# MathsionYang/Ransac

Measured on NVIDIA B200. Metric: hypothesis x point evaluations/s (useful, whole job); ms per robust fit in config, higher is better.
Workload: dtype f32

## Files before the change

### ransac_b200/csrc/common.cuh

```cuda
#pragma once
#include <cuda_runtime.h>
#include <stdint.h>

#include "../../include/usac_gpu.h"

#define USAC_REC_STRIDE 32
#define USAC_TILE_PAIRS 128
#ifndef USAC_WARP_STAGES
#define USAC_WARP_STAGES 2
#endif
#define USAC_SCORE_THREADS 128
#ifndef USAC_SCORE_MIN_CTAS
#define USAC_SCORE_MIN_CTAS 4
#endif
#ifndef USAC_SCORE_GRID_CTAS
#define USAC_SCORE_GRID_CTAS USAC_SCORE_MIN_CTAS
#endif
#ifndef USAC_SQ_MIN_CTAS
#define USAC_SQ_MIN_CTAS 5
#endif
#ifndef USAC_PPI
#define USAC_PPI 4
#endif

enum { REC_MODEL = 0, REC_HINV = 9, REC_BAND = 18, REC_THR = 22 };

struct ProblemDesc {
    int n;
    int n_pairs;
    long long aos_off;
    long long pair_off;
    float mx1, my1, mx2, my2;
    int neigh_type, knn;
    long long knn_off;
    long long grid_off;
    long long cell_start_off;
    long long growth_off, term_off, pool_off;
    long long cursor_off;
    unsigned long long pn_len;
};

__host__ __device__ __forceinline__ unsigned long long pnapsac_length(const ProblemDesc& pd) {
    return pd.pn_len ? pd.pn_len : 20ull * (unsigned long long)pd.n;
}

struct FitState {
    float best_model[9];
    int best_cnt;
    float best_sum;
    long long best_hyp;
    int best_midx;
    unsigned iters, max_iters, samples_drawn, rounds;
    int done;
    int round_pending;
    unsigned long long evals, useful_evals;
    unsigned prosac_t, prosac_n, prosac_largest, prosac_term_len;
    unsigned prosac_t_next, prosac_n_next, prosac_largest_next;
    double sprt_eps, sprt_delta, sprt_A;
    unsigned sprt_cursor;
    int sprt_last_update, sprt_ntests;
};

#define CUDA_TRY(ctx, expr)                                                                         \
    do {                                                                                            \
        cudaError_t _e = (expr);                                                                    \
        if (_e != cudaSuccess) { (ctx)->set_error(#expr, cudaGetErrorString(_e)); return USAC_ERR_CUDA; } \
    } while (0)

__host__ __device__ __forceinline__ int usac_sample_size(int est) {
    return est == USAC_EST_LINE2D ? 2 : est == USAC_EST_HOMOGRAPHY ? 4 : est == USAC_EST_FUNDAMENTAL ? 7 : 5;
}
__host__ __device__ __forceinline__ int usac_models_per_sample(int est) { return est == USAC_EST_FUNDAMENTAL ? 3 : 1; }
__host__ __device__ __forceinline__ constexpr int usac_point_dim(int est) { return est == USAC_EST_LINE2D ? 2 : 4; }

__host__ __device__ __forceinline__ void philox4x32_10(uint32_t c0, uint32_t c1, uint32_t c2, uint32_t c3, uint32_t k0, uint32_t k1, uint32_t out[4]) {
#pragma unroll
    for (int r = 0; r < 10; r++) {
        const uint64_t p0 = (uint64_t)0xD2511F53u * c0, p1 = (uint64_t)0xCD9E8D57u * c2;
        const uint32_t n0 = (uint32_t)(p1 >> 32) ^ c1 ^ k0, n1 = (uint32_t)p1, n2 = (uint32_t)(p0 >> 32) ^ c3 ^ k1, n3 = (uint32_t)p0;
        c0 = n0; c1 = n1; c2 = n2; c3 = n3;
        k0 += 0x9E3779B9u; k1 += 0xBB67AE85u;
    }
    out[0] = c0; out[1] = c1; out[2] = c2; out[3] = c3;
}

__host__ __device__ __forceinline__ void philox_unique(uint64_t seed, uint64_t hyp, uint32_t stream, int n, int m, int* out) {
    uint32_t w[8];
    for (int blk = 0; blk * 4 < m; blk++)
        philox4x32_10((uint32_t)hyp, (uint32_t)(hyp >> 32), (uint32_t)blk, stream, (uint32_t)seed, (uint32_t)(seed >> 32), w + 4 * blk);
    int sorted[8];
    for (int i = 0; i < m; i++) {
        int j = (int)(((uint64_t)w[i] * (uint64_t)(uint32_t)(n - i)) >> 32);
        int pos = 0;
        while (pos < i && j >= sorted[pos]) { j++; pos++; }
        for (int q = i; q > pos; q--) sorted[q] = sorted[q - 1];
        sorted[pos] = j;
        out[i] = j;
    }
}

__device__ __forceinline__ unsigned long long score_key(int cnt, float sum) {
    const unsigned s = (sum > 0.f) ? __float_as_uint(sum) : 0u;
// ... 3 lines not shown
```

### ransac_b200/csrc/score.cuh

```cuda
#pragma once
#include "strict_math.cuh"

__device__ __forceinline__ float fast_rcp(float x) { float r; asm("rcp.approx.ftz.f32 %0, %1;" : "=f"(r) : "f"(x)); return r; }
__device__ __forceinline__ float fast_sqrt(float x) { float r; asm("sqrt.approx.ftz.f32 %0, %1;" : "=f"(r) : "f"(x)); return r; }
__device__ __forceinline__ float fast_rsqrt(float x) { float r; asm("rsqrt.approx.ftz.f32 %0, %1;" : "=f"(r) : "f"(x)); return r; }
__device__ __forceinline__ float2 dup(float x) { return make_float2(x, x); }
__device__ __forceinline__ float abs_max_nan(float a, float b) { float r; asm("max.NaN.f32 %0, %1, %2;" : "=f"(r) : "f"(fabsf(a)), "f"(fabsf(b))); return r; }

__device__ __forceinline__ uint32_t smem_u32(const void* p) { return (uint32_t)__cvta_generic_to_shared(p); }
__device__ __forceinline__ void mbar_init(uint64_t* bar, uint32_t count) {
    asm volatile("mbarrier.init.shared::cta.b64 [%0], %1;" ::"r"(smem_u32(bar)), "r"(count));
}
__device__ __forceinline__ void mbar_expect_tx(uint64_t* bar, uint32_t bytes) {
    asm volatile("mbarrier.arrive.expect_tx.shared::cta.b64 _, [%0], %1;" ::"r"(smem_u32(bar)), "r"(bytes) : "memory");
}
__device__ __forceinline__ bool mbar_try_wait(uint64_t* bar, uint32_t parity) {
    uint32_t ok;
    asm volatile(
        "{\n\t.reg .pred p;\n\t"
        "mbarrier.try_wait.parity.shared::cta.b64 p, [%1], %2;\n\t"
        "selp.u32 %0, 1, 0, p;\n\t}"
        : "=r"(ok)
        : "r"(smem_u32(bar)), "r"(parity)
        : "memory");
    return ok != 0;
}
__device__ __forceinline__ void mbar_wait(uint64_t* bar, uint32_t parity) {
    while (!mbar_try_wait(bar, parity)) {}
}
__device__ __forceinline__ void bulk_copy_g2s(void* dst_smem, const void* src_gmem, uint32_t bytes, uint64_t* bar) {
    asm volatile("cp.async.bulk.shared::cluster.global.mbarrier::complete_tx::bytes [%0], [%1], %2, [%3];" ::"r"(smem_u32(dst_smem)),
                 "l"(src_gmem), "r"(bytes), "r"(smem_u32(bar))
                 : "memory");
}


template <int EST> struct FastModel;

template <> struct FastModel<USAC_EST_HOMOGRAPHY> {
    static constexpr bool WEIGHTED = false;
    float a11, a12, a13, a21, a22, a23, h31, h32, h33;
    float b11, b12, b13, b21, b22, b23, g31, g32, g33;
    float negT, k1, k2;
    __device__ __forceinline__ void load(const float* r) {
        a11 = -r[0]; a12 = -r[1]; a13 = -r[2]; a21 = -r[3]; a22 = -r[4]; a23 = -r[5]; h31 = r[6]; h32 = r[7]; h33 = r[8];
        b11 = -r[9]; b12 = -r[10]; b13 = -r[11]; b21 = -r[12]; b22 = -r[13]; b23 = -r[14]; g31 = r[15]; g32 = r[16]; g33 = r[17];
        negT = -2.f * r[REC_THR]; k1 = r[REC_BAND]; k2 = r[REC_BAND + 1];
        T2p = 2.f * r[REC_THR] * 1.0000019f;
    }
    static constexpr bool TWO_PHASE = true;
    float T2p;
    struct P1 { float2 sa, nz; };
    __device__ __forceinline__ void phase1(const float4 A, const float4 B, P1& s) const {
        const float2 X1 = make_float2(A.x, A.y), Y1 = make_float2(A.z, A.w), X2 = make_float2(B.x, B.y), Y2 = make_float2(B.z, B.w);
        const float2 nz = __ffma2_rn(dup(h31), X1, __ffma2_rn(dup(h32), Y1, dup(h33)));
        const float2 nx = __ffma2_rn(dup(a11), X1, __ffma2_rn(dup(a12), Y1, dup(a13)));
        const float2 ny = __ffma2_rn(dup(a21), X1, __ffma2_rn(dup(a22), Y1, dup(a23)));
        const float2 ax = __ffma2_rn(X2, nz, nx), ay = __ffma2_rn(Y2, nz, ny);
        s.sa = __ffma2_rn(ay, ay, __fmul2_rn(ax, ax));
        s.nz = nz;
    }
    __device__ __forceinline__ void sure(const P1& s, bool& ox, bool& oy) const {
        const float2 az = make_float2(fabsf(s.nz.x), fabsf(s.nz.y));
        const float2 c = __ffma2_rn(dup(T2p), az, dup(k1));
        const float2 c2 = __fmul2_rn(c, c);
        ox = s.sa.x > c2.x; oy = s.sa.y > c2.y;
    }
    __device__ __forceinline__ void phase2(const float4 A, const float4 B, const P1& s, float2& t, float2& band) const {
        const float2 X1 = make_float2(A.x, A.y), Y1 = make_float2(A.z, A.w), X2 = make_float2(B.x, B.y), Y2 = make_float2(B.z, B.w);
        const float2 r1 = make_float2(fabsf(fast_rcp(s.nz.x)), fabsf(fast_rcp(s.nz.y)));
        const float2 d1 = __fmul2_rn(make_float2(fast_sqrt(s.sa.x), fast_sqrt(s.sa.y)), r1);
        const float2 mz = __ffma2_rn(dup(g31), X2, __ffma2_rn(dup(g32), Y2, dup(g33)));
        const float2 mx = __ffma2_rn(dup(b11), X2, __ffma2_rn(dup(b12), Y2, dup(b13)));
        const float2 my = __ffma2_rn(dup(b21), X2, __ffma2_rn(dup(b22), Y2, dup(b23)));
        const float2 r2 = make_float2(fast_rcp(mz.x), fast_rcp(mz.y));
        const float2 ex = __ffma2_rn(mx, r2, X1), ey = __ffma2_rn(my, r2, Y1);
        const float2 sb = __ffma2_rn(ey, ey, __fmul2_rn(ex, ex));
        const float2 d2 = make_float2(fast_sqrt(sb.x), fast_sqrt(sb.y));
        t = __fadd2_rn(__fadd2_rn(d1, dup(negT)), d2);
        const float2 p2 = __fmul2_rn(dup(k2), r2);
        band = __ffma2_rn(dup(k1), r1, make_float2(fabsf(p2.x), fabsf(p2.y)));
    }
    __device__ __forceinline__ void eval(const float4 A, const float4 B, float2& t, float2& s, float2& w) const {
        P1 st;
        bool ox, oy;
        phase1(A, B, st);
        sure(st, ox, oy);
        phase2(A, B, st, t, s);
        if (ox) { t.x = 1.f; s.x = 0.f; }
        if (oy) { t.y = 1.f; s.y = 0.f; }
        w = t;
    }
    __device__ __forceinline__ float2 reject(const float4 A, const float4 B, float2& bound) const {
        const float2 X1 = make_float2(A.x, A.y), Y1 = make_float2(A.z, A.w), X2 = make_float2(B.x, B.y), Y2 = make_float2(B.z, B.w);
        const float2 nz = __ffma2_rn(dup(h31), X1, __ffma2_rn(dup(h32), Y1, dup(h33)));
        const float2 nx = __ffma2_rn(dup(a11), X1, __ffma2_rn(dup(a12), Y1, dup(a13)));
        const float2 ny = __ffma2_rn(dup(a21), X1, __ffma2_rn(dup(a22), Y1, dup(a23)));
        const float2 ax = __ffma2_rn(X2, nz, nx), ay = __ffma2_rn(Y2, nz, ny);
        bound = __ffma2_rn(dup(T2p), make_float2(fabsf(nz.x), fabsf(nz.y)), dup(k1));
        return make_float2(abs_max_nan(ax.x, ay.x), abs_max_nan(ax.y, ay.y));
    }
    static __device__ __forceinline__ float finish(float sum_em, int cnt, float thr) { return 0.5f * (sum_em + (float)cnt * (2.f * thr)); }
    static __device__ __forceinline__ float strict_to_em(float err, float thr) { return 2.f * err - 2.f * thr; }
};

template <> struct FastModel<USAC_EST_FUNDAMENTAL> {
#ifdef USAC_F_SINGLE_PHASE
    static constexpr bool TWO_PHASE = false;
#else
    static constexpr bool TWO_PHASE = true;
#endif
    static constexpr bool WEIGHTED = true;
    float f11, f12, f13, f21, f22, f23, f31, f32, f33, negthr, b1, b0, negthrP, b0P;
    __device__ __forceinline__ void load(const float* r) {
        f11 = r[0]; f12 = r[1]; f13 = r[2]; f21 = r[3]; f22 = r[4]; f23 = r[5]; f31 = r[6]; f32 = r[7]; f33 = r[8];
        negthr = -r[REC_THR]; b1 = r[REC_BAND]; b0 = r[REC_BAND + 1];
        negthrP = -(r[REC_THR] + b1) * 1.0000039f;
        b0P = b0 * 1.0000039f + 1e-37f;
    }
    struct P1 { float2 n2, den; };
    __device__ __forceinline__ void phase1(const float4 A, const float4 B, P1& s) const {
        const float2 X1 = make_float2(A.x, A.y), Y1 = make_float2(A.z, A.w), X2 = make_float2(B.x, B.y), Y2 = make_float2(B.z, B.w);
        const float2 a = __ffma2_rn(dup(f11), X1, __ffma2_rn(dup(f12), Y1, dup(f13)));
        const float2 b = __ffma2_rn(dup(f21), X1, __ffma2_rn(dup(f22), Y1, dup(f23)));
        const float2 c = __ffma2_rn(dup(f11), X2, __ffma2_rn(dup(f21), Y2, dup(f31)));
        const float2 d = __ffma2_rn(dup(f12), X2, __ffma2_rn(dup(f22), Y2, dup(f32)));
        const float2 n = __ffma2_rn(X2, a, __ffma2_rn(Y2, b, __ffma2_rn(dup(f31), X1, __ffma2_rn(dup(f32), Y1, dup(f33)))));
        s.n2 = __fmul2_rn(n, n);
        s.den = __ffma2_rn(d, d, __ffma2_rn(c, c, __ffma2_rn(b, b, __fmul2_rn(a, a))));
    }
    __device__ __forceinline__ void sure(const P1& s, bool& ox, bool& oy) const {
        const float2 u = __ffma2_rn(dup(negthrP), s.den, s.n2);
        ox = u.x > b0P; oy = u.y > b0P;
    }
    __device__ __forceinline__ void phase2(const float4, const float4, const P1& s, float2& t, float2& band) const {
        t = __ffma2_rn(dup(negthr), s.den, s.n2);
        band = __ffma2_rn(dup(b1), s.den, dup(b0));
    }
    __device__ __forceinline__ float2 weight(const P1& s) const { return make_float2(fast_rcp(s.den.x), fast_rcp(s.den.y)); }
    __device__ __forceinline__ float2 reject(const float4 A, const float4 B, float2& bound) const {
        bound = make_float2(0.f, 0.f);
        const float2 X1 = make_float2(A.x, A.y), Y1 = make_float2(A.z, A.w), X2 = make_float2(B.x, B.y), Y2 = make_float2(B.z, B.w);
        const float2 a = __ffma2_rn(dup(f11), X1, __ffma2_rn(dup(f12), Y1, dup(f13)));
        const float2 b = __ffma2_rn(dup(f21), X1, __ffma2_rn(dup(f22), Y1, dup(f23)));
        const float2 c = __ffma2_rn(dup(f11), X2, __ffma2_rn(dup(f21), Y2, dup(f31)));
        const float2 d = __ffma2_rn(dup(f12), X2, __ffma2_rn(dup(f22), Y2, dup(f32)));
        const float2 cp = __ffma2_rn(dup(f31), X1, __ffma2_rn(dup(f32), Y1, dup(f33)));
        const float2 n = __ffma2_rn(X2, a, __ffma2_rn(Y2, b, cp));
        const float2 den = __ffma2_rn(d, d, __ffma2_rn(c, c, __ffma2_rn(b, b, __fmul2_rn(a, a))));
        return __ffma2_rn(dup(negthrP), den, __ffma2_rn(n, n, dup(-b0P)));
    }
    __device__ __forceinline__ void eval(const float4 A, const float4 B, float2& t, float2& s, float2& w) const {
        P1 st;
        phase1(A, B, st);
        phase2(A, B, st, t, s);
        w = weight(st);
    }
    static __device__ __forceinline__ float finish(float sum_em, int cnt, float thr) { return sum_em + (float)cnt * thr; }
    static __device__ __forceinline__ float strict_to_em(float err, float thr) { return err - thr; }
};

template <> struct FastModel<USAC_EST_ESSENTIAL> {
    static constexpr bool WEIGHTED = false;
    float e11, e12, e13, e21, e22, e23, e31, e32, e33, negT, ka, kb, k0, negka, C2;
    __device__ __forceinline__ void load(const float* r) {
        e11 = r[0]; e12 = r[1]; e13 = r[2]; e21 = r[3]; e22 = r[4]; e23 = r[5]; e31 = r[6]; e32 = r[7]; e33 = r[8];
        negT = -2.f * r[REC_THR]; ka = r[REC_BAND]; kb = r[REC_BAND + 1]; k0 = r[REC_BAND + 2];
        negka = -ka;
        const float c = (2.f * r[REC_THR] + k0) * 1.0000039f;
        C2 = c * c * 1.0000039f;
    }
    __device__ __forceinline__ float2 reject(const float4 A, const float4 B, float2& bound) const {
        bound = make_float2(0.f, 0.f);
        const float2 X1 = make_float2(A.x, A.y), Y1 = make_float2(A.z, A.w), X2 = make_float2(B.x, B.y), Y2 = make_float2(B.z, B.w);
        const float2 l1 = __ffma2_rn(dup(e11), X2, __ffma2_rn(dup(e21), Y2, dup(e31)));
        const float2 l2 = __ffma2_rn(dup(e12), X2, __ffma2_rn(dup(e22), Y2, dup(e32)));
        const float2 l3 = __ffma2_rn(dup(e13), X2, __ffma2_rn(dup(e23), Y2, dup(e33)));
        const float2 a1 = __ffma2_rn(l1, X1, __ffma2_rn(l2, Y1, l3));
        const float2 a2 = __ffma2_rn(l2, l2, __fmul2_rn(l1, l1));
        const float2 v = __fadd2_rn(make_float2(fabsf(a1.x), fabsf(a1.y)), dup(negka));
        const float2 m = __fmul2_rn(dup(C2), a2);
        return __ffma2_rn(v, make_float2(fabsf(v.x), fabsf(v.y)), make_float2(-m.x, -m.y));
    }
// ... 422 lines not shown
```

### ransac_b200/csrc/score_sq.cuh

```cuda
#pragma once
#include "score.cuh"

#ifndef USAC_SQ_TRIPVOTE
#define USAC_SQ_TRIPVOTE 2
#endif
#ifndef USAC_SQ_PREFETCH
#define USAC_SQ_PREFETCH 0
#endif
#define USAC_SQ_LANE_CAP 16
#define USAC_SQ_FIXED_BITS 36
#define USAC_SQ_LO_BITS 22

__device__ __forceinline__ void sq_push(bool pred, uint32_t& qaddr, uint32_t entry) {
    asm volatile(
        "{\n\t.reg .pred p;\n\t"
        "setp.ne.u32 p, %1, 0;\n\t"
        "@p st.shared.u32 [%0], %2;\n\t"
        "@p add.u32 %0, %0, 128;\n\t}"
        : "+r"(qaddr)
        : "r"((uint32_t)pred), "r"(entry));
}

template <int EST>
__device__ __noinline__ void sq_drain(const uint32_t* __restrict__ q, uint32_t cnt, uint32_t* pre, const float* __restrict__ recs_group,
                                      const float* __restrict__ aos, int n, double scale, uint32_t* mcnt, uint32_t* mlo, uint32_t* mhi) {
    const int lane = threadIdx.x & 31;
    uint32_t incl = cnt;
#pragma unroll
    for (int o = 1; o < 32; o <<= 1) { const uint32_t y = __shfl_up_sync(0xffffffffu, incl, o); if (lane >= o) incl += y; }
    const uint32_t total = __shfl_sync(0xffffffffu, incl, 31);
    pre[lane] = incl - cnt;
    __syncwarp();
    for (uint32_t base = 0; base < total; base += 64) {
        int l[2], idx[2];
        bool on[2];
        float4 p[2];
#pragma unroll
        for (int h = 0; h < 2; h++) {
            const uint32_t t = base + 32u * h + lane;
            on[h] = t < total;
            l[h] = 0; idx[h] = 0;
            if (on[h]) {
                int ll = 0;
#pragma unroll
                for (int step = 16; step; step >>= 1) if (pre[ll + step] <= t) ll += step;
                l[h] = ll;
                idx[h] = (int)q[(t - pre[ll]) * 32 + ll];
                on[h] = idx[h] < n;
            }
            p[h] = make_float4(0.f, 0.f, 0.f, 0.f);
            if (on[h]) {
                if (EST == USAC_EST_LINE2D) { const float2 v = reinterpret_cast<const float2*>(aos)[idx[h]]; p[h] = make_float4(v.x, v.y, 0.f, 0.f); }
                else p[h] = reinterpret_cast<const float4*>(aos)[idx[h]];
            }
        }
#pragma unroll
        for (int h = 0; h < 2; h++) {
            if (!on[h]) continue;
            const float* rec = recs_group + (size_t)l[h] * USAC_REC_STRIDE;
            const float err = strict_error<EST>(rec, p[h].x, p[h].y, p[h].z, p[h].w);
            if (err < rec[REC_THR]) {
                const unsigned long long fix = __double2ull_rn((double)err * scale);
                atomicAdd(&mcnt[l[h]], 1u);
                atomicAdd(&mlo[l[h]], (uint32_t)(fix & ((1u << USAC_SQ_LO_BITS) - 1u)));
                atomicAdd(&mhi[l[h]], (uint32_t)(fix >> USAC_SQ_LO_BITS));
            }
        }
    }
}

template <int EST>
__global__ void __launch_bounds__(USAC_SCORE_THREADS, USAC_SQ_MIN_CTAS) score_sq_kernel(const ScoreArgs a) {
    constexpr int PAIR_FLOATS = (EST == USAC_EST_LINE2D) ? 4 : 8;
    constexpr int NWARPS = USAC_SCORE_THREADS / 32;
    static_assert(USAC_SQ_LANE_CAP >= 4 * USAC_PPI, "a lane's queue must hold two trips of pushes");
    __shared__ __align__(128) float tile_all[NWARPS][USAC_WARP_STAGES][USAC_TILE_PAIRS * PAIR_FLOATS];
    __shared__ __align__(8) uint64_t full_all[NWARPS][USAC_WARP_STAGES];
    __shared__ __align__(128) uint32_t queue_all[NWARPS][USAC_SQ_LANE_CAP * 32];
    __shared__ uint32_t macc_all[NWARPS][4][32];

    const int lane = threadIdx.x & 31, warp = threadIdx.x >> 5;
    float (*tile)[USAC_TILE_PAIRS * PAIR_FLOATS] = tile_all[warp];
    uint64_t* full = full_all[warp];
    uint32_t* queue = queue_all[warp];
    uint32_t* mcnt = macc_all[warp][0];
    uint32_t* mlo = macc_all[warp][1];
    uint32_t* mhi = macc_all[warp][2];
    uint32_t* pre = macc_all[warp][3];
    const uint32_t q_first = smem_u32(queue) + 4u * (uint32_t)lane;
    const uint32_t q_limit = q_first + 128u * (USAC_SQ_LANE_CAP - 2 * USAC_PPI);
    if (lane == 0) {
#pragma unroll
        for (int s = 0; s < USAC_WARP_STAGES; s++) mbar_init(&full[s], 1);
        asm volatile("fence.mbarrier_init.release.cluster;" ::: "memory");
        asm volatile("fence.proxy.async.shared::cta;" ::: "memory");
    }
    __syncwarp();

    const int mgroups = a.mblocks * NWARPS;
    const unsigned total = a.items ? *a.item_count : (unsigned)a.slots * (unsigned)a.nchunks * (unsigned)mgroups;
    uint32_t g = 0;

    unsigned pending = 0;
    if (USAC_SQ_PREFETCH && lane == 0) pending = atomicAdd(a.work, 1u) - a.work_base;
    for (;;) {
        if (!USAC_SQ_PREFETCH && lane == 0) pending = atomicAdd(a.work, 1u) - a.work_base;
        const unsigned item = __shfl_sync(0xffffffffu, pending, 0);
        int slot, chunk, mgroup;
        if (!score_item(a, item, total, mgroups, slot, chunk, mgroup)) break;
        if (USAC_SQ_PREFETCH && lane == 0) pending = atomicAdd(a.work, 1u) - a.work_base;
        const int M = a.mvalid ? a.mvalid[slot] : a.M;
        if (mgroup * 32 >= M) continue;
        const ProblemDesc pd = a.prob[a.active ? a.active[slot] : slot];
        const int m = mgroup * 32 + lane;
        const bool live = m < M;
        const float* recs_group = a.recs + ((size_t)slot * a.mstride + (size_t)mgroup * 32) * USAC_REC_STRIDE;
        const float* rec = recs_group + (size_t)(live ? lane : 0) * USAC_REC_STRIDE;
        const size_t out = ((size_t)slot * a.nchunks + chunk) * a.mstride + m;

        const int pair_begin = chunk * a.chunk_pairs;
        const int npairs = min(pair_begin + a.chunk_pairs, pd.n_pairs) - pair_begin;
        if (npairs <= 0) {
            if (live) { a.part_cnt[out] = 0; a.part_sum[out] = 0.f; }
            continue;
        }
        const int ntiles = (npairs + USAC_TILE_PAIRS - 1) / USAC_TILE_PAIRS;
        const float* src = a.pairs + ((size_t)pd.pair_off + pair_begin) * PAIR_FLOATS;

        if (lane == 0) {
            asm volatile("fence.proxy.async.shared::cta;" ::: "memory");
            for (int k = 0; k < USAC_WARP_STAGES && k < ntiles; k++) {
                const int s = (g + k) % USAC_WARP_STAGES;
                const uint32_t bytes = min(USAC_TILE_PAIRS, npairs - k * USAC_TILE_PAIRS) * PAIR_FLOATS * 4;
                mbar_expect_tx(&full[s], bytes);
                bulk_copy_g2s(tile[s], src + (size_t)k * USAC_TILE_PAIRS * PAIR_FLOATS, bytes, &full[s]);
            }
        }
        mcnt[lane] = 0u; mlo[lane] = 0u; mhi[lane] = 0u;
        uint32_t acc_cnt = 0;
        unsigned long long acc_sum = 0;
        __syncwarp();

        FastModel<EST> fm;
        fm.load(rec);
        const float thr = rec[REC_THR];
        const double scale = (double)(1ull << USAC_SQ_FIXED_BITS) / (double)thr;
        const float* aos = a.aos + (size_t)pd.aos_off * (EST == USAC_EST_LINE2D ? 2 : 4);
        uint32_t qaddr = q_first;

        auto drain = [&]() {
            asm volatile("" ::: "memory");
            __syncwarp();
            sq_drain<EST>(queue, (qaddr - q_first) >> 7, pre, recs_group, aos, pd.n, scale, mcnt, mlo, mhi);
            __syncwarp();
            acc_cnt += mcnt[lane];
            acc_sum += ((unsigned long long)mhi[lane] << USAC_SQ_LO_BITS) + mlo[lane];
            mcnt[lane] = 0u; mlo[lane] = 0u; mhi[lane] = 0u;
            qaddr = q_first;
            __syncwarp();
        };

        for (int k = 0; k < ntiles; k++) {
            const int s = (g + k) % USAC_WARP_STAGES;
            mbar_wait(&full[s], ((g + k) / USAC_WARP_STAGES) & 1);
            const int np = min(USAC_TILE_PAIRS, npairs - k * USAC_TILE_PAIRS);
            const float4* tp = reinterpret_cast<const float4*>(tile[s]);
            uint32_t ebase = (uint32_t)(2 * (pair_begin + k * USAC_TILE_PAIRS));
            auto load_pair = [&](int j, float4& A, float4& B) {
                if (EST == USAC_EST_LINE2D) { A = tp[j]; B = A; }
                else { A = tp[2 * j]; B = tp[2 * j + 1]; }
            };
            int j = 0;
#pragma unroll 1
            for (; j + USAC_PPI <= np; j += USAC_PPI) {
                float2 z[USAC_PPI], zb[USAC_PPI];
#pragma unroll
                for (int q = 0; q < USAC_PPI; q++) {
                    float4 A, B;
                    load_pair(j + q, A, B);
                    z[q] = fm.reject(A, B, zb[q]);
                }
                bool lane_any = false;
#pragma unroll
                for (int q = 0; q < USAC_PPI; q++) lane_any = lane_any || !(z[q].x > zb[q].x) || !(z[q].y > zb[q].y);
                if (!USAC_SQ_TRIPVOTE || (EST != USAC_EST_HOMOGRAPHY && USAC_SQ_TRIPVOTE == 2) || __any_sync(0xffffffffu, lane_any && live)) {
#pragma unroll
                    for (int q = 0; q < USAC_PPI; q++) {
                        sq_push(!(z[q].x > zb[q].x) && live, qaddr, ebase + 2 * q);
                        sq_push(!(z[q].y > zb[q].y) && live, qaddr, ebase + 2 * q + 1);
                    }
                    if (__any_sync(0xffffffffu, qaddr > q_limit)) drain();
                }
                ebase += 2 * USAC_PPI;
            }
            if (j < np) {
                const int rest = np - j;
#pragma unroll
                for (int q = 0; q < USAC_PPI; q++) {
                    if (q < rest) {
                        float4 A, B;
                        load_pair(j + q, A, B);
                        float2 zb;
                        const float2 z = fm.reject(A, B, zb);
                        sq_push(!(z.x > zb.x) && live, qaddr, ebase + 2 * q);
                        sq_push(!(z.y > zb.y) && live, qaddr, ebase + 2 * q + 1);
                    }
                }
                if (__any_sync(0xffffffffu, qaddr > q_limit)) drain();
            }
            __syncwarp();
            if (lane == 0 && k + USAC_WARP_STAGES < ntiles) {
                asm volatile("fence.proxy.async.shared::cta;" ::: "memory");
                const int nk = k + USAC_WARP_STAGES;
                const uint32_t bytes = min(USAC_TILE_PAIRS, npairs - nk * USAC_TILE_PAIRS) * PAIR_FLOATS * 4;
                mbar_expect_tx(&full[s], bytes);
                bulk_copy_g2s(tile[s], src + (size_t)nk * USAC_TILE_PAIRS * PAIR_FLOATS, bytes, &full[s]);
            }
        }
        g += (uint32_t)ntiles;
        if (__any_sync(0xffffffffu, qaddr != q_first)) drain();
        if (live) {
            a.part_cnt[out] = (int)acc_cnt;
            a.part_sum[out] = (float)((double)acc_sum / scale);
        }
        __syncwarp();
    }
}
```

### ransac_b200/csrc/usac_gpu.cu

```cuda
#include <dlfcn.h>

#include <cub/device/device_radix_sort.cuh>
#include <cub/device/device_scan.cuh>

#include <algorithm>
#include <chrono>
#include <cmath>
#include <cstdio>
#include <cstdlib>
#include <cstring>
#include <map>
#include <string>
#include <thread>
#include <tuple>
#include <vector>

#include "essential.cuh"
#include "pipeline.cuh"
#include "score.cuh"
#include "score_sq.cuh"
#include "sprt.cuh"
#include "refit.cuh"
#include "lo.cuh"
#include "knn.cuh"
// ... 543 lines not shown
    CUDA_TRY(c, cudaStreamSynchronize(c->stream));
    *k_out = d.knn;
    return USAC_OK;
}

extern "C" int usac_gpu_set_pnapsac_length(usac_gpu_ctx* c, int problem, unsigned long long local_samples) {
    if (!c || problem < 0 || problem >= c->P) return fail(c, USAC_ERR_ARG, "set_pnapsac_length: bad arguments");
    cudaSetDevice(c->device);
    c->h_prob[problem].pn_len = local_samples;
    return push_desc(c);
}

extern "C" int usac_gpu_set_neighbors_grid(usac_gpu_ctx* c, int problem, int cell_size) {
    if (!c || problem < 0 || problem >= c->P || cell_size <= 0) return fail(c, USAC_ERR_ARG, "set_neighbors_grid: bad arguments");
    if (usac_point_dim(c->est) != 4) return fail(c, USAC_ERR_ARG, "set_neighbors_grid: needs correspondences (nearest_neighbors.cpp:172 reads 4 columns)");
    cudaSetDevice(c->device);
    ProblemDesc& d = c->h_prob[problem];
    const int n = d.n;
    SideUsed& u = c->side;
    CUDA_TRY(c, reserve_segment(c->d_cell_of_point, u.grid, (size_t)n, c->stream));
    CUDA_TRY(c, reserve_segment(c->d_members, u.grid, (size_t)n, c->stream));
    CUDA_TRY(c, reserve_segment(c->d_rank, u.grid, (size_t)n, c->stream));
    CUDA_TRY(c, reserve_segment(c->d_cell_start, u.cell_start, (size_t)n + 1, c->stream));
    CUDA_TRY(c, c->d_grid_keys.ensure(2 * (size_t)n));
    CUDA_TRY(c, c->d_grid_ints.ensure(4 * (size_t)n + 1));
    struct { unsigned long long* p; } keys{c->d_grid_keys.p}, skeys{c->d_grid_keys.p + n};
    struct { int* p; } idx{c->d_grid_ints.p}, sidx{c->d_grid_ints.p + n}, flags{c->d_grid_ints.p + 2 * (size_t)n}, cellid1{c->d_grid_ints.p + 3 * (size_t)n},
        ovf{c->d_grid_ints.p + 4 * (size_t)n};
    CUDA_TRY(c, cudaMemsetAsync(ovf.p, 0, sizeof(int), c->stream));
    const int g = (n + 255) / 256;
    grid_keys_kernel<<<g, 256, 0, c->stream>>>(c->d_aos.p + (size_t)d.aos_off * 4, n, (float)cell_size, keys.p, idx.p, ovf.p);
    size_t tb1 = 0, tb2 = 0;
    cub::DeviceRadixSort::SortPairs(nullptr, tb1, keys.p, skeys.p, idx.p, sidx.p, n, 0, 64, c->stream);
    cub::DeviceScan::InclusiveSum(nullptr, tb2, flags.p, cellid1.p, n, c->stream);
    CUDA_TRY(c, c->d_grid_temp.ensure(std::max(tb1, tb2)));
    struct { unsigned char* p; } temp{c->d_grid_temp.p};
    size_t tb = std::max(tb1, tb2);
    CUDA_TRY(c, cub::DeviceRadixSort::SortPairs(temp.p, tb, keys.p, skeys.p, idx.p, sidx.p, n, 0, 64, c->stream));
    grid_flags_kernel<<<g, 256, 0, c->stream>>>(skeys.p, n, flags.p);
    tb = std::max(tb1, tb2);
    CUDA_TRY(c, cub::DeviceScan::InclusiveSum(temp.p, tb, flags.p, cellid1.p, n, c->stream));
    int* cs = c->d_cell_start.p + u.cell_start;
    grid_fill_tail_kernel<<<(n + 1 + 255) / 256, 256, 0, c->stream>>>(cellid1.p, n, cs);
    grid_starts_kernel<<<g, 256, 0, c->stream>>>(flags.p, cellid1.p, n - 0, cs);
    grid_scatter_kernel<<<g, 256, 0, c->stream>>>(sidx.p, cellid1.p, cs, n, c->d_cell_of_point.p + u.grid, c->d_members.p + u.grid, c->d_rank.p + u.grid);
    int h_ovf = 0;
    CUDA_TRY(c, cudaMemcpyAsync(&h_ovf, ovf.p, sizeof(int), cudaMemcpyDeviceToHost, c->stream));
    CUDA_TRY(c, cudaStreamSynchronize(c->stream));
    CUDA_TRY(c, cudaGetLastError());
    if (h_ovf) return fail(c, USAC_ERR_ARG, "set_neighbors_grid: cell coordinates exceed 16 bits (cell_size too small for this coordinate range)");
    d.grid_off = (long long)u.grid;
    d.cell_start_off = (long long)u.cell_start;
    u.grid += (size_t)n;
    u.cell_start += (size_t)n + 1;
    if (d.cursor_off < 0) CUDA_TRY(c, append_segment(c->d_cursors, u.cursors, (const unsigned*)nullptr, 3 * (size_t)n + 1, &d.cursor_off, c->stream));
    d.neigh_type = USAC_NEIGH_GRID;
    return push_desc(c);
}

extern "C" int usac_gpu_set_sprt_pool(usac_gpu_ctx* c, int problem, const int* pool) {
    if (!c || problem < 0 || problem >= c->P || !pool) return fail(c, USAC_ERR_ARG, "set_sprt_pool: bad arguments");
    cudaSetDevice(c->device);
    SideUsed& u = c->side;
    ProblemDesc& d = c->h_prob[problem];
    for (int i = 0; i < d.n; i++) if (pool[i] < 0 || pool[i] >= d.n) return fail(c, USAC_ERR_ARG, "set_sprt_pool: index out of range");
    CUDA_TRY(c, append_segment(c->d_pool, u.pool, pool, (size_t)d.n, &d.pool_off, c->stream));
    const int dim = usac_point_dim(c->est);
    CUDA_TRY(c, c->d_pool_pts.ensure((size_t)c->total_points * dim));
    pool_gather_kernel<<<(d.n + 255) / 256, 256, 0, c->stream>>>(c->d_aos.p + (size_t)d.aos_off * dim, c->d_pool.p + d.pool_off, d.n, dim,
                                                                  c->d_pool_pts.p + (size_t)d.aos_off * dim);
    CUDA_TRY(c, cudaGetLastError());
    c->h_pool_set[problem] = 1;
    return push_desc(c);
}

static void launch_score(usac_gpu_ctx* c, ScoreArgs a, int slots, int mblocks, bool dense_survivors = false) {
    a.mblocks = mblocks; a.slots = slots;
    constexpr int warps_per_cta = USAC_SCORE_THREADS / 32;
    const long long items = (long long)slots * a.nchunks * mblocks * warps_per_cta;
    const unsigned grid = (unsigned)std::min<long long>((items + warps_per_cta - 1) / warps_per_cta,
                                                        (long long)c->prop.multiProcessorCount * USAC_SCORE_GRID_CTAS);
    static const int legacy = [] { const char* e = getenv("USAC_GPU_SCORE_LEGACY"); return e ? atoi(e) : 0; }();
    const bool loop_kernel = legacy == 1 || c->est == USAC_EST_LINE2D || (dense_survivors && legacy != 2);
    unsigned grid_ctas = grid;
    if (a.items) {
        grid_ctas = (unsigned)c->prop.multiProcessorCount * (loop_kernel ? USAC_SCORE_GRID_CTAS : USAC_SQ_MIN_CTAS);
        a.work = c->d_item_count.p + 1; a.work_base = 0;
    } else {
        if (!loop_kernel) grid_ctas = (unsigned)std::min<long long>((items + warps_per_cta - 1) / warps_per_cta, (long long)c->prop.multiProcessorCount * USAC_SQ_MIN_CTAS);
        a.work = c->d_work.p; a.work_base = c->work_next;
        c->work_next += (unsigned)items + grid_ctas * warps_per_cta;
    }
    auto& ev = c->next_score_event();
    cudaEventRecord(ev.first, c->stream);
    if (loop_kernel) {
        switch (c->est) {
            case USAC_EST_LINE2D: score_kernel<USAC_EST_LINE2D><<<grid_ctas, USAC_SCORE_THREADS, 0, c->stream>>>(a); break;
            case USAC_EST_HOMOGRAPHY: score_kernel<USAC_EST_HOMOGRAPHY><<<grid_ctas, USAC_SCORE_THREADS, 0, c->stream>>>(a); break;
            case USAC_EST_FUNDAMENTAL: score_kernel<USAC_EST_FUNDAMENTAL><<<grid_ctas, USAC_SCORE_THREADS, 0, c->stream>>>(a); break;
            default: score_kernel<USAC_EST_ESSENTIAL><<<grid_ctas, USAC_SCORE_THREADS, 0, c->stream>>>(a); break;
        }
    } else {
        switch (c->est) {
            case USAC_EST_HOMOGRAPHY: score_sq_kernel<USAC_EST_HOMOGRAPHY><<<grid_ctas, USAC_SCORE_THREADS, 0, c->stream>>>(a); break;
            case USAC_EST_FUNDAMENTAL: score_sq_kernel<USAC_EST_FUNDAMENTAL><<<grid_ctas, USAC_SCORE_THREADS, 0, c->stream>>>(a); break;
            default: score_sq_kernel<USAC_EST_ESSENTIAL><<<grid_ctas, USAC_SCORE_THREADS, 0, c->stream>>>(a); break;
        }
    }
    if (!a.items && cudaPeekAtLastError() != cudaSuccess) c->work_next = a.work_base;
    cudaEventRecord(ev.second, c->stream);
    c->last_launches++;
    c->last_score_launches++;
}

static void plan_chunks(const usac_gpu_ctx* c, int slots, int mblocks, int max_pairs, int* chunk_pairs, int* nchunks) {
    static const int per_warp = [] { const char* e = getenv("USAC_GPU_ITEMS_PER_WARP"); const int v = e ? atoi(e) : 0; return v > 0 ? v : 16; }();
    const long long warps = (long long)c->prop.multiProcessorCount * std::max(USAC_SCORE_GRID_CTAS, USAC_SQ_MIN_CTAS) * (USAC_SCORE_THREADS / 32);
    const long long base = (long long)slots * mblocks * (USAC_SCORE_THREADS / 32);
    static const int min_tiles_env = [] { const char* e = getenv("USAC_GPU_MIN_TILES"); return e ? atoi(e) : 0; }();
    const int min_tiles = min_tiles_env > 0 ? min_tiles_env : (max_pairs >= 65536 ? 8 : 2);
    const int max_chunks = std::min(65535, std::max(1, max_pairs / (min_tiles * USAC_TILE_PAIRS)));
    int nc = (int)std::min<long long>((per_warp * warps + base - 1) / base, max_chunks);
    nc = std::max(nc, 1);
    int cp = (max_pairs + nc - 1) / nc;
    cp = ((cp + 1) / 2) * 2;
    nc = (max_pairs + cp - 1) / cp;
    *chunk_pairs = cp;
    *nchunks = std::max(nc, 1);
}

static void collect_timing(usac_gpu_ctx* c) {
    float ms = 0;
    cudaEventElapsedTime(&ms, c->ev0, c->ev1);
    c->last_total_ms = ms;
    float s = 0;
    for (size_t i = 0; i < c->score_events_used; i++) {
        float t = 0;
        cudaEventElapsedTime(&t, c->score_events[i].first, c->score_events[i].second);
        s += t;
    }
    c->last_score_ms = s;
}

__global__ void __launch_bounds__(256) final_reduce_kernel(const int* __restrict__ part_cnt, const float* __restrict__ part_sum, int M, int mstride,
                                                           int nchunks, int* __restrict__ cnt, float* __restrict__ sum) {
    __shared__ int s_c[8][32];
    __shared__ float s_s[8][32];
    const int lane = threadIdx.x & 31, warp = threadIdx.x >> 5;
    const int q = blockIdx.x * 32 + lane;
    int cc = 0;
    float s = 0.f;
    if (q < M)
        for (int ch = warp; ch < nchunks; ch += 8) { cc += part_cnt[(size_t)ch * mstride + q]; s += part_sum[(size_t)ch * mstride + q]; }
    s_c[warp][lane] = cc;
    s_s[warp][lane] = s;
    __syncthreads();
    if (warp != 0 || q >= M) return;
    cc = 0; s = 0.f;
    for (int w = 0; w < 8; w++) { cc += s_c[w][lane]; s += s_s[w][lane]; }
    cnt[q] = cc;
    sum[q] = s;
}

extern "C" int usac_gpu_score(usac_gpu_ctx* c, int problem, const float* models, int M, float threshold, int* inliers_out, float* sumerr_out) {
    if (!c || problem < 0 || problem >= c->P || !models || M < 0 || !(threshold > 0.f)) return fail(c, USAC_ERR_ARG, "score: bad arguments");
    if (M == 0) return USAC_OK;
    cudaSetDevice(c->device);
    const int w = c->est == USAC_EST_LINE2D ? 3 : 9;
    CUDA_TRY(c, c->d_q_models.ensure((size_t)M * w));
    CUDA_TRY(c, c->d_q_recs.ensure((size_t)M * USAC_REC_STRIDE));
    const ProblemDesc& d = c->h_prob[problem];
    const int mblocks = (M + USAC_SCORE_THREADS - 1) / USAC_SCORE_THREADS;
    int chunk_pairs, nchunks;
    plan_chunks(c, 1, mblocks, d.n_pairs, &chunk_pairs, &nchunks);
    CUDA_TRY(c, c->d_part_cnt.ensure((size_t)nchunks * M));
    CUDA_TRY(c, c->d_part_sum.ensure((size_t)nchunks * M));
    CUDA_TRY(c, c->d_q_cnt.ensure(M));
    CUDA_TRY(c, c->d_q_sum.ensure(M));
    c->score_events_used = 0; c->last_launches = 0; c->last_score_launches = 0;
    cudaEventRecord(c->ev0, c->stream);
    CUDA_TRY(c, cudaMemcpyAsync(c->d_q_models.p, models, sizeof(float) * w * M, cudaMemcpyHostToDevice, c->stream));
    c->h_active[0] = problem;
    CUDA_TRY(c, cudaMemcpyAsync(c->d_active.p, c->h_active, sizeof(int), cudaMemcpyHostToDevice, c->stream));
    prepare_models_kernel<<<(M + 127) / 128, 128, 0, c->stream>>>(c->est, c->d_q_models.p, M, w, threshold, c->d_prob.p, problem, c->d_q_recs.p);
    c->last_launches++;
    ScoreArgs a{};
    a.pairs = c->d_pairs.p; a.aos = c->d_aos.p; a.prob = c->d_prob.p; a.active = c->d_active.p; a.recs = c->d_q_recs.p; a.mvalid = nullptr;
// ... 1510 lines not shown
```

Before: 1158 billion.

## Add transposed queue scoring kernel for homography with pairs held in registers

Adds a homography-only score kernel that swaps the loop order. Each lane keeps several point pairs in registers and loops over the warp's 32 models, reading each model's reject coefficients from shared memory staged per warp. Survivors go into a queue of (pair, model) entries, and the drain reads the model index from the entry. The goal is to cut global pair loads per model and to skip pushes with a warp vote when no lane survives. In exchange it adds shared-memory staging, a doubled queue entry size and higher occupancy targets (8 CTAs), which may pressure registers. It also removes the tripvote option from the existing queue kernel.

```diff
diff --git a/ransac_b200/csrc/common.cuh b/ransac_b200/csrc/common.cuh
--- a/ransac_b200/csrc/common.cuh
+++ b/ransac_b200/csrc/common.cuh
@@ -18,6 +18,12 @@
 #endif
 #ifndef USAC_SQ_MIN_CTAS
 #define USAC_SQ_MIN_CTAS 5
+#endif
+#ifndef USAC_SQT_MIN_CTAS
+#define USAC_SQT_MIN_CTAS 8
+#endif
+#ifndef USAC_SQT_PAIRS
+#define USAC_SQT_PAIRS 4
 #endif
 #ifndef USAC_PPI
 #define USAC_PPI 4
diff --git a/ransac_b200/csrc/score.cuh b/ransac_b200/csrc/score.cuh
--- a/ransac_b200/csrc/score.cuh
+++ b/ransac_b200/csrc/score.cuh
@@ -99,6 +99,16 @@
         const float2 ax = __ffma2_rn(X2, nz, nx), ay = __ffma2_rn(Y2, nz, ny);
         bound = __ffma2_rn(dup(T2p), make_float2(fabsf(nz.x), fabsf(nz.y)), dup(k1));
         return make_float2(abs_max_nan(ax.x, ay.x), abs_max_nan(ax.y, ay.y));
+    }
+    static constexpr int REJECT_FLOATS = 12;
+    __device__ __forceinline__ void stage_reject(float* c) const {
+        reinterpret_cast<float4*>(c)[0] = make_float4(a11, a12, a13, a21);
+        reinterpret_cast<float4*>(c)[1] = make_float4(a22, a23, h31, h32);
+        reinterpret_cast<float4*>(c)[2] = make_float4(h33, T2p, k1, 0.f);
+    }
+    __device__ __forceinline__ void load_reject(const float* c) {
+        const float4 u = reinterpret_cast<const float4*>(c)[0], v = reinterpret_cast<const float4*>(c)[1], w = reinterpret_cast<const float4*>(c)[2];
+        a11 = u.x; a12 = u.y; a13 = u.z; a21 = u.w; a22 = v.x; a23 = v.y; h31 = v.z; h32 = v.w; h33 = w.x; T2p = w.y; k1 = w.z;
     }
     static __device__ __forceinline__ float finish(float sum_em, int cnt, float thr) { return 0.5f * (sum_em + (float)cnt * (2.f * thr)); }
     static __device__ __forceinline__ float strict_to_em(float err, float thr) { return 2.f * err - 2.f * thr; }
diff --git a/ransac_b200/csrc/score_sq.cuh b/ransac_b200/csrc/score_sq.cuh
--- a/ransac_b200/csrc/score_sq.cuh
+++ b/ransac_b200/csrc/score_sq.cuh
@@ -1,9 +1,6 @@
 #pragma once
 #include "score.cuh"
 
-#ifndef USAC_SQ_TRIPVOTE
-#define USAC_SQ_TRIPVOTE 2
-#endif
 #ifndef USAC_SQ_PREFETCH
 #define USAC_SQ_PREFETCH 0
 #endif
@@ -21,8 +18,8 @@
         : "r"((uint32_t)pred), "r"(entry));
 }
 
-template <int EST>
-__device__ __noinline__ void sq_drain(const uint32_t* __restrict__ q, uint32_t cnt, uint32_t* pre, const float* __restrict__ recs_group,
+template <int EST, typename Entry>
+__device__ __noinline__ void sq_drain(const Entry* __restrict__ q, uint32_t cnt, uint32_t* pre, const float* __restrict__ recs_group,
                                       const float* __restrict__ aos, int n, double scale, uint32_t* mcnt, uint32_t* mlo, uint32_t* mhi) {
     const int lane = threadIdx.x & 31;
     uint32_t incl = cnt;
@@ -44,8 +41,9 @@
                 int ll = 0;
 #pragma unroll
                 for (int step = 16; step; step >>= 1) if (pre[ll + step] <= t) ll += step;
-                l[h] = ll;
-                idx[h] = (int)q[(t - pre[ll]) * 32 + ll];
+                const Entry e = q[(t - pre[ll]) * 32 + ll];
+                if constexpr (sizeof(Entry) == 8) { idx[h] = (int)e.x; l[h] = (int)e.y; }
+                else { idx[h] = (int)e; l[h] = ll; }
                 on[h] = idx[h] < n;
             }
             p[h] = make_float4(0.f, 0.f, 0.f, 0.f);
@@ -180,17 +178,12 @@
                     load_pair(j + q, A, B);
                     z[q] = fm.reject(A, B, zb[q]);
                 }
-                bool lane_any = false;
-#pragma unroll
-                for (int q = 0; q < USAC_PPI; q++) lane_any = lane_any || !(z[q].x > zb[q].x) || !(z[q].y > zb[q].y);
-                if (!USAC_SQ_TRIPVOTE || (EST != USAC_EST_HOMOGRAPHY && USAC_SQ_TRIPVOTE == 2) || __any_sync(0xffffffffu, lane_any && live)) {
-#pragma unroll
-                    for (int q = 0; q < USAC_PPI; q++) {
-                        sq_push(!(z[q].x > zb[q].x) && live, qaddr, ebase + 2 * q);
-                        sq_push(!(z[q].y > zb[q].y) && live, qaddr, ebase + 2 * q + 1);
-                    }
-                    if (__any_sync(0xffffffffu, qaddr > q_limit)) drain();
-                }
+#pragma unroll
+                for (int q = 0; q < USAC_PPI; q++) {
+                    sq_push(!(z[q].x > zb[q].x) && live, qaddr, ebase + 2 * q);
+                    sq_push(!(z[q].y > zb[q].y) && live, qaddr, ebase + 2 * q + 1);
+                }
+                if (__any_sync(0xffffffffu, qaddr > q_limit)) drain();
                 ebase += 2 * USAC_PPI;
             }
             if (j < np) {
@@ -226,3 +219,139 @@
         __syncwarp();
     }
 }
+
+__device__ __forceinline__ void sq_push_pm(float z, float bound, uint32_t& qaddr, uint32_t idx, uint32_t m) {
+    asm volatile(
+        "{\n\t.reg .pred p;\n\t"
+        "setp.leu.f32 p, %1, %2;\n\t"
+        "@p st.shared.v2.u32 [%0], {%3, %4};\n\t"
+        "@p add.u32 %0, %0, 256;\n\t}"
+        : "+r"(qaddr)
+        : "f"(z), "f"(bound), "r"(idx), "r"(m));
+}
+
+template <int V> struct SqtInt { static constexpr int value = V; };
+
+template <int EST>
+__global__ void __launch_bounds__(USAC_SCORE_THREADS, USAC_SQT_MIN_CTAS) score_sqt_kernel(const ScoreArgs a) {
+    static_assert(EST == USAC_EST_HOMOGRAPHY, "the transposed queue kernel is built for the homography only");
+    using FM = FastModel<EST>;
+    constexpr int NWARPS = USAC_SCORE_THREADS / 32;
+    constexpr int P = USAC_SQT_PAIRS;
+    static_assert(USAC_SQ_LANE_CAP >= 4 * P, "a lane's queue must hold two model-trips of pushes");
+    __shared__ __align__(16) float coef_all[NWARPS][32][FM::REJECT_FLOATS];
+    __shared__ __align__(256) uint2 queue_all[NWARPS][USAC_SQ_LANE_CAP * 32];
+    __shared__ uint32_t macc_all[NWARPS][4][32];
+
+    const int lane = threadIdx.x & 31, warp = threadIdx.x >> 5;
+    float (*coef)[FM::REJECT_FLOATS] = coef_all[warp];
+    uint2* queue = queue_all[warp];
+    uint32_t* mcnt = macc_all[warp][0];
+    uint32_t* mlo = macc_all[warp][1];
+    uint32_t* mhi = macc_all[warp][2];
+    uint32_t* pre = macc_all[warp][3];
+    const uint32_t q_first = smem_u32(queue) + 8u * (uint32_t)lane;
+    const uint32_t q_limit = q_first + 256u * (USAC_SQ_LANE_CAP - 2 * P);
+
+    const int mgroups = a.mblocks * NWARPS;
+    const unsigned total = a.items ? *a.item_count : (unsigned)a.slots * (unsigned)a.nchunks * (unsigned)mgroups;
+    for (;;) {
+        unsigned item = 0;
+        if (lane == 0) item = atomicAdd(a.work, 1u) - a.work_base;
+        item = __shfl_sync(0xffffffffu, item, 0);
+        int slot, chunk, mgroup;
+        if (!score_item(a, item, total, mgroups, slot, chunk, mgroup)) break;
+        const int M = a.mvalid ? a.mvalid[slot] : a.M;
+        if (mgroup * 32 >= M) continue;
+        const ProblemDesc pd = a.prob[a.active ? a.active[slot] : slot];
+        const int nm = min(32, M - mgroup * 32);
+        const bool live = lane < nm;
+        const float* recs_group = a.recs + ((size_t)slot * a.mstride + (size_t)mgroup * 32) * USAC_REC_STRIDE;
+        const float* rec = recs_group + (size_t)(live ? lane : 0) * USAC_REC_STRIDE;
+        const size_t out = ((size_t)slot * a.nchunks + chunk) * a.mstride + mgroup * 32 + lane;
+
+        const int pair_begin = chunk * a.chunk_pairs;
+        const int npairs = min(pair_begin + a.chunk_pairs, pd.n_pairs) - pair_begin;
+        if (npairs <= 0) {
+            if (live) { a.part_cnt[out] = 0; a.part_sum[out] = 0.f; }
+            continue;
+        }
+        {
+            FM fm;
+            fm.load(rec);
+            if (live) fm.stage_reject(coef[lane]);
+        }
+        mcnt[lane] = 0u; mlo[lane] = 0u; mhi[lane] = 0u;
+        uint32_t acc_cnt = 0;
+        unsigned long long acc_sum = 0;
+        const float thr = rec[REC_THR];
+        const double scale = (double)(1ull << USAC_SQ_FIXED_BITS) / (double)thr;
+        const float* aos = a.aos + (size_t)pd.aos_off * 4;
+        const float4* src = reinterpret_cast<const float4*>(a.pairs + ((size_t)pd.pair_off + pair_begin) * 8);
+        uint32_t qaddr = q_first;
+        __syncwarp();
+
+        auto drain = [&]() {
+            asm volatile("" ::: "memory");
+            __syncwarp();
+            sq_drain<EST>(queue, (qaddr - q_first) >> 8, pre, recs_group, aos, pd.n, scale, mcnt, mlo, mhi);
+            __syncwarp();
+            acc_cnt += mcnt[lane];
+            acc_sum += ((unsigned long long)mhi[lane] << USAC_SQ_LO_BITS) + mlo[lane];
+            mcnt[lane] = 0u; mlo[lane] = 0u; mhi[lane] = 0u;
+            qaddr = q_first;
+            __syncwarp();
+        };
+
+        auto block = [&](auto pp, auto check, const int j0) {
+            constexpr int PP = decltype(pp)::value;
+            constexpr bool CHECK = decltype(check)::value;
+            const uint32_t e0 = 2u * (uint32_t)(pair_begin + j0 + lane);
+            int m = 0;
+            while (m < nm) {
+                float4 A[PP], B[PP];
+                bool v[PP];
+#pragma unroll
+                for (int q = 0; q < PP; q++) {
+                    const int j = j0 + 32 * q + lane;
+                    v[q] = !CHECK || j < npairs;
+                    A[q] = make_float4(0.f, 0.f, 0.f, 0.f); B[q] = A[q];
+                    if (v[q]) { A[q] = __ldg(src + 2 * j); B[q] = __ldg(src + 2 * j + 1); }
+                }
+                bool full = false;
+#pragma unroll 1
+                for (; m < nm && !full; m++) {
+                    FM f;
+                    f.load_reject(coef[m]);
+                    float2 z[PP], zb[PP];
+#pragma unroll
+                    for (int q = 0; q < PP; q++) {
+                        z[q] = f.reject(A[q], B[q], zb[q]);
+                        if (CHECK && !v[q]) { z[q] = make_float2(INFINITY, INFINITY); zb[q] = make_float2(0.f, 0.f); }
+                    }
+                    bool lane_any = false;
+#pragma unroll
+                    for (int q = 0; q < PP; q++) lane_any = lane_any || !(z[q].x > zb[q].x) || !(z[q].y > zb[q].y);
+                    if (__any_sync(0xffffffffu, lane_any)) {
+#pragma unroll
+                        for (int q = 0; q < PP; q++) {
+                            sq_push_pm(z[q].x, zb[q].x, qaddr, e0 + 64u * q, (uint32_t)m);
+                            sq_push_pm(z[q].y, zb[q].y, qaddr, e0 + 64u * q + 1u, (uint32_t)m);
+                        }
+                        full = __any_sync(0xffffffffu, qaddr > q_limit);
+                    }
+                }
+                if (full) drain();
+            }
+        };
+        int j0 = 0;
+        for (; j0 + 32 * P <= npairs; j0 += 32 * P) block(SqtInt<P>{}, SqtInt<false>{}, j0);
+        for (; j0 < npairs; j0 += 32) block(SqtInt<1>{}, SqtInt<true>{}, j0);
+        if (__any_sync(0xffffffffu, qaddr != q_first)) drain();
+        if (live) {
+            a.part_cnt[out] = (int)acc_cnt;
+            a.part_sum[out] = (float)((double)acc_sum / scale);
+        }
+        __syncwarp();
+    }
+}
diff --git a/ransac_b200/csrc/usac_gpu.cu b/ransac_b200/csrc/usac_gpu.cu
--- a/ransac_b200/csrc/usac_gpu.cu
+++ b/ransac_b200/csrc/usac_gpu.cu
@@ -649,12 +649,13 @@
                                                         (long long)c->prop.multiProcessorCount * USAC_SCORE_GRID_CTAS);
     static const int legacy = [] { const char* e = getenv("USAC_GPU_SCORE_LEGACY"); return e ? atoi(e) : 0; }();
     const bool loop_kernel = legacy == 1 || c->est == USAC_EST_LINE2D || (dense_survivors && legacy != 2);
+    const int queue_ctas = c->est == USAC_EST_HOMOGRAPHY ? USAC_SQT_MIN_CTAS : USAC_SQ_MIN_CTAS;
     unsigned grid_ctas = grid;
     if (a.items) {
-        grid_ctas = (unsigned)c->prop.multiProcessorCount * (loop_kernel ? USAC_SCORE_GRID_CTAS : USAC_SQ_MIN_CTAS);
+        grid_ctas = (unsigned)c->prop.multiProcessorCount * (loop_kernel ? USAC_SCORE_GRID_CTAS : queue_ctas);
         a.work = c->d_item_count.p + 1; a.work_base = 0;
     } else {
-        if (!loop_kernel) grid_ctas = (unsigned)std::min<long long>((items + warps_per_cta - 1) / warps_per_cta, (long long)c->prop.multiProcessorCount * USAC_SQ_MIN_CTAS);
+        if (!loop_kernel) grid_ctas = (unsigned)std::min<long long>((items + warps_per_cta - 1) / warps_per_cta, (long long)c->prop.multiProcessorCount * queue_ctas);
         a.work = c->d_work.p; a.work_base = c->work_next;
         c->work_next += (unsigned)items + grid_ctas * warps_per_cta;
     }
@@ -669,7 +670,7 @@
         }
     } else {
         switch (c->est) {
-            case USAC_EST_HOMOGRAPHY: score_sq_kernel<USAC_EST_HOMOGRAPHY><<<grid_ctas, USAC_SCORE_THREADS, 0, c->stream>>>(a); break;
+            case USAC_EST_HOMOGRAPHY: score_sqt_kernel<USAC_EST_HOMOGRAPHY><<<grid_ctas, USAC_SCORE_THREADS, 0, c->stream>>>(a); break;
             case USAC_EST_FUNDAMENTAL: score_sq_kernel<USAC_EST_FUNDAMENTAL><<<grid_ctas, USAC_SCORE_THREADS, 0, c->stream>>>(a); break;
             default: score_sq_kernel<USAC_EST_ESSENTIAL><<<grid_ctas, USAC_SCORE_THREADS, 0, c->stream>>>(a); break;
         }
```

New measurement: 1302 billion, median of 6. 12.5% higher.
